# sekulas/vRod

Measured on AMD Instinct MI355X. Metric: queries/sec + recall@10 vs CPU ref, 10M×768 cosine, batch=1024, 1/2/4/8 GPU, higher is better.
Workload: dtype bf16

## Files before the change

### vrod_amd/csrc/kernels_select.hip

```cpp
#include "vrod_common.h"
#include "vrod_kernels.h"

namespace vrod {

constexpr int kSortThreads = 1024;

template <uint32_t NT = kSortThreads>
__device__ __forceinline__ void bitonic_sort_desc(uint64_t* __restrict__ a, uint32_t n) {
    const uint32_t tid = threadIdx.x, lane = tid & 63, wave = tid >> 6;
    constexpr uint32_t kWaves = NT / 64;
    const uint32_t W = n / 128 < kWaves ? (n / 128 ? n / 128 : 1) : kWaves;
    const uint32_t S = n / W;
    const bool active = wave < W;
    bool dirty_local = false;
    for (uint32_t k = 2; k <= n; k <<= 1) {
        for (uint32_t j = k >> 1; j > 0; j >>= 1) {
            if (j >= S) {
                if (dirty_local) { __syncthreads(); dirty_local = false; }
                for (uint32_t t = tid; t < (n >> 1); t += NT) {
                    const uint32_t i = 2 * t - (t & (j - 1));
                    const uint32_t l = i + j;
                    const bool up = (i & k) == 0;
                    const uint64_t x = a[i], y = a[l];
                    if ((x < y) == up) { a[i] = y; a[l] = x; }
                }
                __syncthreads();
            } else {
                if (active) {
                    const uint32_t base = wave * S;
                    for (uint32_t t = lane; t < (S >> 1); t += 64) {
                        const uint32_t i = base + 2 * t - (t & (j - 1));
                        const uint32_t l = i + j;
                        const bool up = (i & k) == 0;
                        const uint64_t x = a[i], y = a[l];
// ... 150 lines not shown
    const int lane = threadIdx.x & 63;
    for (uint32_t off = threadIdx.x; off < kCompactSlice; off += 256) {
        const uint64_t i = i0 + off;
        uint32_t skey = 0;
        bool take = false;
        if (i < n && !(row_mask && ((row_mask[i >> 5] >> (i & 31u)) & 1u))) {
            skey = score_key<METRIC>(sc[i]);
            take = skey >= thr_key;
        }
        const unsigned long long m = __ballot(take);
        if (m) {
            uint32_t base = 0;
            if (lane == 0) base = atomicAdd(&cnt[q], (uint32_t)__popcll(m));
            base = __shfl(base, 0);
            if (take) {
                const uint32_t pos = base + (uint32_t)__popcll(m & ((1ull << lane) - 1ull));
                if (pos < cap) keys[(uint64_t)q * cap + pos] = make_key(skey, (uint32_t)i);
            }
        }
    }
}

void launch_hist_compact(const float* d_scores, uint64_t score_ld, uint64_t n, int nq, int metric,
                         const uint32_t* d_hist, int hist_bits, uint32_t kp, uint64_t* d_keys,
                         uint32_t cap, uint32_t* d_cnt, uint32_t* d_status, const uint32_t* d_row_mask, hipStream_t s) {
    dim3 grid((unsigned)((n + kCompactSlice - 1) / kCompactSlice), nq);
    if (metric == M_COSINE)
        hist_compact_kernel<M_COSINE><<<grid, 256, 0, s>>>(d_scores, score_ld, n, d_hist, hist_bits, kp, d_keys, cap, d_cnt, d_status, d_row_mask);
    else
        hist_compact_kernel<M_L2><<<grid, 256, 0, s>>>(d_scores, score_ld, n, d_hist, hist_bits, kp, d_keys, cap, d_cnt, d_status, d_row_mask);
}

constexpr uint32_t kCompactThreads = 256;
__global__ __launch_bounds__(kCompactThreads) void list_compact_kernel(
    uint2* __restrict__ lists, uint32_t* __restrict__ counts, uint32_t cap, int metric,
    uint32_t keep, uint32_t wsize, float* __restrict__ thr, uint32_t* __restrict__ status,
    uint32_t* __restrict__ cand_rows, float* __restrict__ cand_fast, float* __restrict__ T) {
    extern __shared__ __attribute__((aligned(16))) uint64_t win[];
    const uint32_t q = blockIdx.x, tid = threadIdx.x;
    const uint32_t c = counts[q];
    const uint32_t n = c < cap ? c : cap;
    uint2* l = lists + (uint64_t)q * cap;
    const uint32_t kk = keep;
    uint32_t have = 0;
    uint32_t done = 0;
    while (done < n) {
        const uint32_t room = wsize - have;
        const uint32_t take = n - done < room ? n - done : room;
        for (uint32_t i = tid; i < take; i += kCompactThreads) {
            const uint2 e = l[done + i];
            win[have + i] = make_key(score_key_rt(__uint_as_float(e.x), metric), e.y);
        }
        const uint32_t m = have + take;
        const uint32_t np2 = pow2_ceil(m < 2 ? 2 : m);
        for (uint32_t i = m + tid; i < np2; i += kCompactThreads) win[i] = 0ull;
        __syncthreads();
        bitonic_sort_desc<kCompactThreads>(win, np2);
        have = m < kk ? m : kk;
        done += take;
        __syncthreads();
    }
    for (uint32_t i = tid; i < have; i += kCompactThreads) {
        const uint64_t key = win[i];
        l[i] = make_uint2(__float_as_uint(key_to_score_rt(key_skey(key), metric)), key_row(key));
    }
    if (cand_rows) {
        for (uint32_t i = tid; i < keep; i += kCompactThreads) {
            const uint64_t key = i < have ? win[i] : 0ull;
            cand_rows[(uint64_t)q * keep + i] = i < have ? key_row(key) : 0xFFFFFFFFu;
            cand_fast[(uint64_t)q * keep + i] = i < have ? key_to_score_rt(key_skey(key), metric) : __uint_as_float(kScoreNoneBits);
        }
    }
    if (tid == 0) {
        counts[q] = have;
        float t = thr[q];
        if (n >= keep && have >= keep) { t = key_to_score_rt(key_skey(win[keep - 1]), metric); thr[q] = t; }
        if (T) T[q] = t;
        if (c > cap) atomicOr(&status[q], 2u);
    }
}

void launch_list_compact(uint2* d_lists, uint32_t* d_counts, uint32_t cap, int nq, int metric,
                         uint32_t keep, float* d_thr, uint32_t* d_status, uint32_t* d_cand_rows,
                         float* d_cand_fast, float* d_T, hipStream_t s) {
    const uint32_t wsize = keep <= 1024 ? 2048u : kSelectChunk;
    list_compact_kernel<<<nq, kCompactThreads, (size_t)wsize * 8, s>>>(d_lists, d_counts, cap, metric, keep, wsize, d_thr, d_status,
                                                                     d_cand_rows, d_cand_fast, d_T);
}

constexpr uint32_t kSampleListCap = 2048;
template <int METRIC>
__global__ __launch_bounds__(256) void sample_select_kernel(const float* __restrict__ scores, uint64_t score_ld,
                                                            uint32_t n, uint32_t j, float* __restrict__ thr) {
    __shared__ __attribute__((aligned(16))) uint32_t hist[4096];
    __shared__ uint32_t ctl[8];
    const float* sc = scores + (uint64_t)blockIdx.x * score_ld;
    const uint32_t tid = threadIdx.x;
    if (j <= 256) {
        typedef float f4 __attribute__((ext_vector_type(4)));
        const f4 none4 = {__uint_as_float(kScoreNoneBits), __uint_as_float(kScoreNoneBits), __uint_as_float(kScoreNoneBits), __uint_as_float(kScoreNoneBits)};
        const uint32_t n4 = (n + 3) / 4;
        auto load4 = [&](uint32_t i4) -> f4 {
            if (i4 >= n4) return none4;
            f4 v = *reinterpret_cast<const f4*>(sc + (uint64_t)i4 * 4);
            if (i4 * 4 + 3 >= n) {
#pragma unroll
                for (int e = 0; e < 4; ++e) if (i4 * 4 + e >= n) v[e] = __uint_as_float(kScoreNoneBits);
            }
            return v;
        };
        uint32_t best = 0;
        for (uint32_t i0 = 0; i0 < n4; i0 += 256 * 8) {
// ... 89 lines not shown
    }
    if (lane == 0) thr[q] = key_to_score_rt(prefix, METRIC);
}

void launch_sample_select(const float* d_scores, uint64_t score_ld, uint32_t n_sample, int nq,
                          int metric, uint32_t j, float* d_thr, hipStream_t s) {
    if (!nq) return;
    if (n_sample <= kSampleWaveMax && j >= 1) {
        const int grid = (nq + 3) / 4;
        if (metric == M_COSINE) sample_select_wave_kernel<M_COSINE><<<grid, 256, 0, s>>>(d_scores, score_ld, n_sample, j, (uint32_t)nq, d_thr);
        else sample_select_wave_kernel<M_L2><<<grid, 256, 0, s>>>(d_scores, score_ld, n_sample, j, (uint32_t)nq, d_thr);
        return;
    }
    if (metric == M_COSINE) sample_select_kernel<M_COSINE><<<nq, 256, 0, s>>>(d_scores, score_ld, n_sample, j, d_thr);
    else sample_select_kernel<M_L2><<<nq, 256, 0, s>>>(d_scores, score_ld, n_sample, j, d_thr);
}

__global__ __launch_bounds__(256) void mask_sample_kernel(float* __restrict__ scores, uint64_t score_ld, uint32_t n, uint32_t nq,
                                                          uint64_t row0, const uint32_t* __restrict__ row_mask, float worst) {
    const uint32_t c = blockIdx.x * 256 + threadIdx.x;
    if (c >= n) return;
    const uint64_t r = row0 + c;
    if (!((row_mask[r >> 5] >> (r & 31u)) & 1u)) return;
    for (uint32_t q = blockIdx.y; q < nq; q += gridDim.y) scores[(uint64_t)q * score_ld + c] = worst;
}

void launch_mask_sample(float* d_scores, uint64_t score_ld, uint32_t n_sample, int nq, uint64_t row0,
                        const uint32_t* d_row_mask, int metric, hipStream_t s) {
    if (!nq || !n_sample || !d_row_mask) return;
    const dim3 grid((n_sample + 255) / 256, (unsigned)std::min(nq, 64));
    mask_sample_kernel<<<grid, 256, 0, s>>>(d_scores, score_ld, n_sample, (uint32_t)nq, row0, d_row_mask, worst_score(metric));
}

__global__ __launch_bounds__(kSortThreads) void final_topk_kernel(
    const uint32_t* __restrict__ cand_rows, const float* __restrict__ cand_fast,
    const float* __restrict__ cand_canon, const float* __restrict__ T, uint32_t kp, uint32_t k,
    int metric, IdMap idmap, int eps_mode, float eps_c, const uint32_t* __restrict__ max_qn2_bits,
    const uint32_t* __restrict__ max_xn2_bits, uint64_t* __restrict__ out_ids,
    float* __restrict__ out_scores, uint32_t* __restrict__ status, float* __restrict__ max_err) {
    extern __shared__ __attribute__((aligned(16))) uint64_t skeys[];
    const uint32_t q = blockIdx.x;
    const bool small = kp <= kRankSortMax;
    const uint32_t np2 = small ? kp : pow2_ceil(kp);
    float err = 0.0f;
    for (uint32_t i = threadIdx.x; i < np2; i += kSortThreads) {
        uint64_t key = 0;
        if (i < kp) {
            const uint32_t row = cand_rows[(uint64_t)q * kp + i];
            if (row != 0xFFFFFFFFu) {
                const float c = cand_canon[(uint64_t)q * kp + i];
                key = make_key(score_key_rt(c, metric), row);
                float e = __builtin_fabsf(cand_fast[(uint64_t)q * kp + i] - c);
                if (eps_mode == 1) e = e / __builtin_fmaxf(__builtin_fabsf(c), 1e-30f);
                if (e == e) err = __builtin_fmaxf(err, e);
            }
        }
        skeys[i] = key;
    }
    for (int o = 32; o > 0; o >>= 1) err = __builtin_fmaxf(err, __shfl_xor(err, o));
    if ((threadIdx.x & 63) == 0 && err > 0.0f) atomicMax((uint32_t*)max_err, __float_as_uint(err));
    __syncthreads();
    const uint64_t* sorted;
    if (small) {
        rank_sort_desc(skeys, skeys + kRankSortMax, np2);
        sorted = skeys + kRankSortMax;
    } else {
        bitonic_sort_desc(skeys, np2);
        sorted = skeys;
    }
    for (uint32_t i = threadIdx.x; i < k; i += kSortThreads) {
        const uint64_t key = i < np2 ? sorted[i] : 0ull;
        out_ids[(uint64_t)q * k + i] = key ? idmap(key_row(key)) : UINT64_MAX;
        out_scores[(uint64_t)q * k + i] = key ? key_to_score_rt(key_skey(key), metric) : __uint_as_float(kScoreNoneBits);
    }
    if (threadIdx.x == 0) {
        const float t = T[q];
        bool ok;
        const float qn_ = __builtin_sqrtf(__uint_as_float(*max_qn2_bits)), xn_ = __builtin_sqrtf(__uint_as_float(*max_xn2_bits));
        const float span = metric == M_COSINE ? qn_ * xn_ : (qn_ + xn_) * (qn_ + xn_);
        const float span_eps = eps_mode == 1 ? 0.0f : eps_c * span + eps_c * 2.3509887e-38f;
        if (!(span < 3.0e38f) || !(span + span_eps <= 3.4028234663852886e38f)) {
            ok = false;
        } else if (t == worst_score(metric)) {
            ok = true;
        } else {
            const uint64_t kk = (k >= 1 && k <= np2) ? sorted[k - 1] : 0ull;
            if (!kk) {
                ok = false;
            } else {
                const float sk = key_to_score_rt(key_skey(kk), metric);
                const float qn = __builtin_sqrtf(__uint_as_float(*max_qn2_bits));
                const float xn = __builtin_sqrtf(__uint_as_float(*max_xn2_bits));
                const float eps = (eps_mode == 0 ? eps_c * qn * xn
                                 : eps_mode == 1 ? eps_c * __builtin_fabsf(t) + 1e-30f
                                                 : eps_c * (qn + xn) * (qn + xn)) + eps_c * 2.3509887e-38f;
                ok = metric == M_COSINE ? (sk > t + eps) : (sk < t - eps);
            }
        }
        if (!ok) atomicOr(&status[q], 1u);
    }
}

void launch_final_topk(const uint32_t* d_cand_rows, const float* d_cand_fast,
                       const float* d_cand_canon, const float* d_T, int nq, uint32_t kp, uint32_t k,
                       int metric, const IdMap& idmap, int eps_mode, float eps_c,
                       const uint32_t* d_max_qn2_bits, const uint32_t* d_max_xn2_bits,
                       uint64_t* d_out_ids, float* d_out_scores, uint32_t* d_status,
                       float* d_max_err, hipStream_t s) {
    if (!nq) return;
    size_t lds = sort_lds_bytes(kp);
    if (lds < 2 * kRankSortMax * sizeof(uint64_t)) lds = 2 * kRankSortMax * sizeof(uint64_t);
    final_topk_kernel<<<nq, kSortThreads, lds, s>>>(d_cand_rows, d_cand_fast, d_cand_canon, d_T, kp, k, metric, idmap, eps_mode, eps_c, d_max_qn2_bits, d_max_xn2_bits, d_out_ids, d_out_scores, d_status, d_max_err);
}

__global__ __launch_bounds__(256) void gather_readback_kernel(const uint32_t* __restrict__ status, uint32_t nq,
                                                              uint32_t* __restrict__ flags3,
                                                              const uint32_t* __restrict__ max_xn2,
                                                              uint32_t* __restrict__ out) {
    for (uint32_t i = blockIdx.x * 256 + threadIdx.x; i < nq; i += gridDim.x * 256) out[i] = status[i];
    if (blockIdx.x == 0 && threadIdx.x < 4) {
        out[nq + threadIdx.x] = threadIdx.x < 3 ? flags3[threadIdx.x] : *max_xn2;
        if (threadIdx.x < 3) flags3[threadIdx.x] = 0;
    }
}

void launch_gather_readback(const uint32_t* d_status, uint32_t nq, uint32_t* d_flags3, const uint32_t* d_max_xn2,
                            uint32_t* d_out, hipStream_t s) {
    gather_readback_kernel<<<(nq + 255) / 256 > 0 ? (nq + 255) / 256 : 1, 256, 0, s>>>(d_status, nq, d_flags3, d_max_xn2, d_out);
}

__global__ __launch_bounds__(256) void band_prepare_kernel(const uint32_t* __restrict__ qidx, uint32_t nf, uint32_t nf_pad,
                                                           const float* __restrict__ out_scores, uint32_t k, int metric,
                                                           int eps_mode, float eps_c, const uint32_t* __restrict__ max_qn2_bits,
                                                           const uint32_t* __restrict__ max_xn2_bits, const float* __restrict__ qn2_all,
                                                           float* __restrict__ thr, float* __restrict__ qn2, uint32_t* __restrict__ counts,
                                                           uint32_t* __restrict__ ok) {
    const uint32_t f = blockIdx.x * 256 + threadIdx.x;
    if (f >= nf_pad) return;
    const float never = metric == M_COSINE ? __builtin_huge_valf() : -__builtin_huge_valf();
    counts[f] = 0u;
    if (f >= nf) { thr[f] = never; qn2[f] = 0.0f; ok[f] = 0u; return; }
    const uint32_t q = qidx[f];
    qn2[f] = qn2_all[q];
    const float ck = out_scores[(uint64_t)q * k + (k - 1)];
    const float qn = __builtin_sqrtf(__uint_as_float(*max_qn2_bits)), xn = __builtin_sqrtf(__uint_as_float(*max_xn2_bits));
    const float span = metric == M_COSINE ? qn * xn : (qn + xn) * (qn + xn);
    if (!(ck == ck) || !(span < 3.0e38f) || eps_mode == 1) { thr[f] = never; ok[f] = 0u; return; }
    const float eps = (eps_mode == 0 ? eps_c * qn * xn : eps_c * (qn + xn) * (qn + xn)) + eps_c * 2.3509887e-38f;
    const float slack = 1.01f * eps + 1e-37f;
    const float t = metric == M_COSINE ? ck - slack : ck + slack;
    if (!(span + eps <= 3.4028234663852886e38f) || !(__builtin_fabsf(t) <= 3.4028234663852886e38f)) { thr[f] = never; ok[f] = 0u; return; }
    thr[f] = t;
    ok[f] = 1u;
}

void launch_band_prepare(const uint32_t* d_qidx, uint32_t nf, uint32_t nf_pad, const float* d_out_scores, uint32_t k, int metric,
                         int eps_mode, float eps_c, const uint32_t* d_max_qn2_bits, const uint32_t* d_max_xn2_bits,
                         const float* d_qn2_all, float* d_thr, float* d_qn2, uint32_t* d_counts, uint32_t* d_ok, hipStream_t s) {
    if (!nf_pad) return;
    band_prepare_kernel<<<(nf_pad + 255) / 256, 256, 0, s>>>(d_qidx, nf, nf_pad, d_out_scores, k, metric, eps_mode, eps_c, d_max_qn2_bits,
                                                            d_max_xn2_bits, d_qn2_all, d_thr, d_qn2, d_counts, d_ok);
// ... 178 lines not shown
```

### vrod_amd/csrc/search_plan.h

```cpp
#pragma once
#include <stdint.h>

#include <algorithm>
#include <cmath>
#include <vector>

#include "../../include/vrod.h"

namespace vrod {

constexpr uint32_t kRowTile = 256;
constexpr uint32_t kSelectChunk = 8192;
enum : int { M_COSINE = 0, M_L2 = 1 };

inline uint64_t round_up(uint64_t x, uint64_t m) { return (x + m - 1) / m * m; }

inline int score_form(int metric) { return metric == VROD_METRIC_L2 ? M_L2 : M_COSINE; }
inline int prep_form(int metric) { return metric == VROD_METRIC_COSINE ? M_COSINE : M_L2; }

struct Route {
    int path;
    bool split;
};
inline bool can_split(bool split_enabled, int dtype, uint64_t N, uint32_t k) {
// ... 60 lines not shown
        }
    }
    return b;
}
inline float eps_bound(int eps_mode, float eps_c, float qn2, float xn2) {
    const float qn = std::sqrt(qn2), xn = std::sqrt(xn2);
    return (eps_mode == 0 ? eps_c * qn * xn : eps_mode == 1 ? eps_c  : eps_c * (qn + xn) * (qn + xn)) +
           (eps_mode == 1 ? 0.f : eps_c * 2.3509887e-38f);
}

struct SearchPlan {
    int path = 0;
    bool split = false;
    uint32_t kp = 0;
    int eps_mode = 0;
    float eps_c = 0.f;
    uint32_t nq_pad = 0;
    uint64_t N = 0;
};
inline SearchPlan make_plan(int path, bool split, int form, uint32_t dim, uint64_t N, uint32_t nq, uint32_t k, uint32_t kp_boost,
                            uint32_t kp_margin) {
    SearchPlan p;
    p.path = path;
    p.split = split;
    p.kp = choose_kp(path, split, form, N, k, kp_boost, kp_margin);
    const FastBound b = fast_bound(path, split, form, dim);
    p.eps_mode = b.mode;
    p.eps_c = b.c;
    p.nq_pad = (uint32_t)round_up(nq, path == VROD_PATH_MFMA ? 256 : 8);
    p.N = N;
    return p;
}

struct StagePlan { uint32_t S, j; std::vector<uint64_t> bounds; };
inline StagePlan plan_stages(uint64_t N, uint32_t kp, uint32_t cap, uint32_t max_sample_rows, uint64_t stage_growth,
                             uint64_t sample_rows) {
    StagePlan p;
    const uint64_t g_auto = 5;
    const uint64_t g = std::max<uint64_t>(2, std::min<uint64_t>(stage_growth ? stage_growth : g_auto, cap / (3ull * kp)));
    if (sample_rows) max_sample_rows = (uint32_t)std::min<uint64_t>(sample_rows, max_sample_rows);
    uint64_t S = std::min<uint64_t>(N / (g * g), max_sample_rows);
    S = std::max<uint64_t>(S, std::min<uint64_t>(N, std::max<uint64_t>(4ull * kp, kRowTile)));
    S = std::min<uint64_t>(round_up(S, kRowTile), N);
    p.S = (uint32_t)S;
    p.j = (uint32_t)std::min<uint64_t>(kp, S);
    for (uint64_t b = S * g; b < N; b *= g) {
        if (N - b < b / 2) break;
        p.bounds.push_back(b / kRowTile * kRowTile);
    }
    p.bounds.push_back(N);
    return p;
}

struct KpBoost {
    static constexpr uint32_t kMax = 8;
    uint32_t boost = 1, clean = 0, hold = 0;
};
inline void kp_boost_step(KpBoost& s, uint32_t used, bool failures) {
    if (s.hold) --s.hold;
    if (failures) {
        s.clean = 0;
        if (used >= KpBoost::kMax) { s.boost = 1; s.hold = 256; }
        else if (!s.hold && used == s.boost) s.boost *= 2;
    } else if (used == s.boost && ++s.clean >= 64 && s.boost > 1) {
        s.boost /= 2;
        s.clean = 0;
// ... 65 lines not shown
```

### vrod_amd/csrc/vrod_index.hip

```cpp
#include <hip/hip_runtime.h>
#include <dlfcn.h>
#include <fcntl.h>
#include <unistd.h>
#include <rccl/rccl.h>

#include <algorithm>
#include <cmath>
#include <cstdarg>
#include <cstdio>
#include <cstdlib>
#include <cstring>
#include <string>
#include <vector>

#include "../../include/vrod.h"
#include "vrod_common.h"
#include "vrod_kernels.h"
#include "kernels_range.h"
#include "search_plan.h"
#include "compact_plan.h"
#include "label_plan.h"
#include "group_plan.h"
#include "byid_plan.h"

// ... 49 lines not shown
};

constexpr uint32_t kPaceRegions = 8, kPaceWords = 192, kClaimWords = (uint32_t)kMfmaClaimWords;
constexpr size_t kSlotFlagBytes = (64 + kPaceRegions * (kPaceWords + kClaimWords)) * 4;

struct Pending {
    bool active = false;
    bool trivial = false;
    uint32_t nq = 0, k = 0;
    SearchPlan plan{};
    uint64_t* out_ids = nullptr;
    float* out_scores = nullptr;
    hipStream_t stream = nullptr;
    uint32_t* flags = nullptr;
    DevBuf q_raw, q_lp, scores, keys_a, keys_b, lists, small, hist, cand_rows, cand_fast, cand_canon;
    DevBuf q_f32;
    DevBuf dump;
    DevBuf q_planes;
    DevBuf band_idx, band_q, band_q_lp, band_planes, band_small, band_ids, band_scores;
    uint32_t pace_launches = 0;
    uint32_t* h_readback = nullptr;
    size_t h_readback_words = 0;
    hipEvent_t done = nullptr;
    hipEvent_t scans_done = nullptr;
    hipEvent_t mid_done = nullptr;
    bool mid_recorded = false;
    std::vector<hipEvent_t> ev;
    size_t ev_used = 0, t0 = 0, t1 = 0;
    std::vector<std::pair<size_t, size_t>> scan_pairs;
    int sample_pair = -1;
    int tail_pair = -1;
    uint32_t seq = 0;
    bool early_sample = false;
    uint32_t kp_boost_used = 1;
    vrod_search_stats st{};

    struct GraphKey {
        const void *q = nullptr, *oi = nullptr, *os = nullptr, *corpus = nullptr, *xn = nullptr, *mask = nullptr;
        const void* bufs[12] = {};
        uint64_t N = 0, id_offset = 0;
        uint32_t nq = 0, k = 0;
        int path = 0;
        bool operator==(const GraphKey& o) const { return memcmp(this, &o, sizeof *this) == 0; }
    };
    GraphKey gkey{};
    bool gkey_valid = false;
    hipGraphExec_t gexec = nullptr;
    GraphKey gkey_graph{};
    bool graph_off = false;
    SearchPlan g_plan{};
    vrod_search_stats g_st{};
};

struct vrod_index {
    int device = 0;
    int num_cus = 256;
    uint32_t dim = 0, ld = 0;
    int dtype = VROD_DTYPE_F32, metric = VROD_METRIC_COSINE;
    size_t esize = 4;
    uint64_t count = 0, capacity = 0, id_offset = 0;
    void* corpus = nullptr;
    float* xnorm2 = nullptr;
    uint32_t* max_xn2_bits = nullptr;
    hipStream_t stream = nullptr;
    int path = VROD_PATH_AUTO;
    int profiling = 0;
// ... 332 lines not shown
    if (e == hipSuccess) { launch_xn2_max(idx->xnorm2, plan.live, idx->max_xn2_bits, s); e = hipGetLastError(); }
    if (e == hipSuccess) e = hipMemsetAsync(idx->del_dev, 0, cap_words * 4, s);
    if (e == hipSuccess && idx->filter_on) e = hipMemcpyAsync(idx->eff_dev, new_eff.data(), cap_words * 4, hipMemcpyHostToDevice, s);
    if (e == hipSuccess && idx->lab_dev) e = hipMemcpyAsync(idx->lab_dev, new_lab.data(), count * 4, hipMemcpyHostToDevice, s);
    if (e == hipSuccess) e = hipStreamSynchronize(s);
    if (e != hipSuccess)
        return fail(VROD_ERR_HIP, "vrod_index_compact: %s while rows were moving: the handle is unusable, destroy it", hipGetErrorString(e));

    if (out_new_ids) compact_new_ids(del, count, idx->id_offset, out_new_ids);
    std::fill(idx->del_bits.begin(), idx->del_bits.end(), 0u);
    idx->n_deleted = 0;
    idx->count = plan.live;
    if (idx->filter_on) { idx->allow_bits.swap(new_allow); idx->eff_bits.swap(new_eff); }
    if (idx->lab_dev) std::copy(new_lab.begin(), new_lab.end(), idx->lab_bits.begin());
    idx->planes_rows = 0;
    mask_changed(idx);
    return VROD_OK;
}

namespace vrod {
const DebugEnv& debug_env() {
    static const DebugEnv env = [] {
        DebugEnv d;
        auto num = [](const char* name, long long dflt) { const char* e = getenv(name); return e && *e ? atoll(e) : dflt; };
        auto on = [](const char* name) { const char* e = getenv(name); return !e || e[0] != '0'; };
        d.pace_kt = (int)num("VROD_DEBUG_PACE_KT", d.pace_kt);
        d.pace_tiles = (int)num("VROD_DEBUG_PACE", d.pace_tiles);
        d.w4_steal = on("VROD_DEBUG_W4_STEAL");
        d.skinny = on("VROD_DEBUG_SKINNY");
        d.stage_growth = (uint64_t)num("VROD_DEBUG_STAGE_GROWTH", 0);
        d.sample_rows = (uint64_t)num("VROD_DEBUG_SAMPLE_ROWS", 0);
        d.kp_margin = (uint32_t)num("VROD_DEBUG_KP_MARGIN", 0);
        if (const char* e = getenv("VROD_DEBUG_EARLY_SAMPLE")) d.early_sample = e[0] != '0' ? 1 : 0;
        d.sample_grouped = on("VROD_DEBUG_SAMPLE_GROUPED");
        d.graph = on("VROD_DEBUG_GRAPH");
        d.band = on("VROD_DEBUG_BAND");
        return d;
    }();
    return env;
}
}

struct Timer {
    vrod_index* idx;
    Pending& P;
    Timer(vrod_index* i, Pending& p) : idx(i), P(p) {}
    size_t mark() {
        if (idx->profiling < 2) return 0;
        if (P.ev_used == P.ev.size()) {
            hipEvent_t e;
            if (hipEventCreate(&e) != hipSuccess) return 0;
            P.ev.push_back(e);
        }
        (void)hipEventRecord(P.ev[P.ev_used], P.stream);
        return P.ev_used++;
    }
    void arm(size_t& a, size_t& b) {
        a = b = 0;
        if (!idx->profiling) return;
        while (P.ev.size() < P.ev_used + 2) {
            hipEvent_t e;
            if (hipEventCreate(&e) != hipSuccess) return;
            P.ev.push_back(e);
        }
        a = P.ev_used++;
        b = P.ev_used++;
// ... 266 lines not shown
            tm.arm(a, b);
            g_launch_events = LaunchEvents{};
            if (b) HIP_TRY(hipEventRecord(P.ev[a], s));
        }
        launch_rescore_list(idx->corpus, idx->dtype, form, idx->dim, idx->ld, P.q_f32.as<float>() + (size_t)q0 * idx->ld, gc, list, m,
                            P.scores.as<float>(), score_ld, s);
        if (idx->profiling && b) {
            HIP_TRY(hipEventRecord(P.ev[b], s));
            P.scan_pairs.push_back({a, b});
        }
        st.scan_launches++;
        const uint64_t* keys; uint64_t kld, kn;
        VROD_TRY(select_chain(idx, P, P.scores.as<float>(), score_ld, m, (int)gc, kx, nullptr, &keys, &kld, &kn));
        launch_list_keys_to_output(keys, kld, kn, (int)gc, form, k, list, idmap_of(idx), P.out_ids + (size_t)q0 * k,
                                   P.out_scores + (size_t)q0 * k, s);
    }
    VROD_TRY(record_scans_done(P, s));
    st.scan_bytes = (double)m * idx->ld * idx->esize;
    st.scan_flops = 2.0 * nq * (double)m * idx->dim;
    HIP_TRY(hipGetLastError());
    return VROD_OK;
}

static int mfma_pass(vrod_index* idx, Pending& P, Timer& tm, const void* q_lp) {
    const SearchPlan& plan = P.plan;
    const uint64_t N = plan.N;
    const uint32_t nq = P.nq, kp = plan.kp, cap = kSelectChunk;
    const int form = score_form(idx->metric);
    const SmallBlock B = small_block(P);
    const ListBlock L = list_block(P);
    vrod_search_stats& st = P.st;
    hipStream_t s = P.stream;
    const int early_env = debug_env().early_sample;
    const bool early = early_env >= 0 ? early_env == 1 : N <= 6000000ull;
    Pending& O = other_slot(idx, P);
    HIP_TRY(hipStreamWaitEvent(s, early ? O.mid_done : O.scans_done, 0));
    MfmaScanArgs a;
    VROD_TRY(mfma_args(idx, P, a, idx->dtype == VROD_DTYPE_BF16 ? q_lp : P.q_f32.p, B.qn2, B.thr, nq, plan.nq_pad));
    if (plan.split) {
        if (idx->planes_rows < N) {
            launch_split_rows((const float*)idx->corpus + idx->planes_rows * idx->ld, N - idx->planes_rows, idx->ld, idx->ldp,
                              (char*)idx->planes + idx->planes_rows * 2ull * idx->ldp * 2ull, false, s);
            if (round_up(N, kRowTile) > N)
                HIP_TRY(hipMemsetAsync((char*)idx->planes + N * 2ull * idx->ldp * 2ull, 0, (round_up(N, kRowTile) - N) * 2ull * idx->ldp * 2ull, s));
            idx->planes_rows = N;
        }
        VROD_TRY(use_split_planes(idx, a, P.q_f32.as<float>(), plan.nq_pad, P.q_planes, s));
    }
    const int scan_dtype = plan.split ? VROD_DTYPE_BF16 : idx->dtype;
    P.pace_launches = 0;
    std::vector<uint64_t> bounds{N};
    if (N > cap) {
        const uint32_t nqb = plan.nq_pad / 256;
        const StagePlan sp = plan_stages(N, kp, cap, std::max<uint32_t>(1, (uint32_t)idx->num_cus / nqb) * kRowTile,
                                         debug_env().stage_growth, debug_env().sample_rows);
        bounds = sp.bounds;
        MfmaScanArgs d = a;
        const uint64_t w0 = sample_window(idx, sp.S, N);
        d.row_begin = (uint32_t)w0; d.row_end = (uint32_t)(w0 + sp.S);
        const bool group_env = debug_env().sample_grouped && !idx->row_mask();
        const uint32_t grows = group_env ? mfma_dense_group_rows(d, scan_dtype) : 0u;
        const uint32_t n_groups = grows ? (uint32_t)(round_up(sp.S, kRowTile) / grows) : 0u;
        const bool grouped = grows && (uint64_t)sp.j * 8 <= n_groups && sp.S % kRowTile == 0;
        const uint32_t dense_ld = grouped ? (uint32_t)round_up(n_groups, 64) : (uint32_t)round_up(sp.S, kRowTile);
        const uint32_t n_sel = grouped ? n_groups : sp.S;
        VROD_TRY(P.scores.ensure((size_t)plan.nq_pad * dense_ld * 4));
        d.dense_out = P.scores.as<float>(); d.dense_ld = dense_ld; d.dense_grouped = grouped;
        d.pace = pace_region(P, P.pace_launches++); d.pace_is_zero = true;
        size_t e0, e1;
        tm.arm(e0, e1);
        launch_scan_mfma(d, scan_dtype, idx->num_cus, s);
        P.sample_pair = (int)P.scan_pairs.size();
        P.early_sample = early;
        P.scan_pairs.push_back({e0, e1});
        st.scan_launches++;
        launch_mask_sample(P.scores.as<float>(), dense_ld, n_sel, (int)nq, w0, idx->row_mask(), form, s);
        launch_sample_select(P.scores.as<float>(), dense_ld, n_sel, (int)nq, form, sp.j, B.thr, s);
    }
    HIP_TRY(hipStreamWaitEvent(s, early ? O.scans_done : O.done, 0));
    uint64_t lo = 0;
    for (size_t li = 0; li < bounds.size(); ++li) {
        const bool last = li + 1 == bounds.size();
        launch_filtered(idx, P, tm, a, scan_dtype, lo, bounds[li], true, last);
        lo = std::max(lo, bounds[li]);
        if (li + 2 == bounds.size()) { HIP_TRY(hipEventRecord(P.mid_done, s)); P.mid_recorded = true; }
        if (last) VROD_TRY(record_scans_done(P, s));
        launch_list_compact(L.lists, L.counts, cap, (int)nq, form, kp, B.thr, B.status, last ? P.cand_rows.as<uint32_t>() : nullptr,
                            last ? P.cand_fast.as<float>() : nullptr, last ? B.T : nullptr, s);
    }
    HIP_TRY(hipGetLastError());
    return VROD_OK;
}

static int search_enqueue_body(vrod_index* idx, Pending& P, const float* d_queries_raw, uint32_t nq, uint32_t k,
                               uint64_t* d_out_ids, float* d_out_scores, bool in_graph) {
    vrod_search_stats& st = P.st;
    st = vrod_search_stats{};
    st.nq = nq;
    st.k = k;
    P.nq = nq; P.k = k; P.out_ids = d_out_ids; P.out_scores = d_out_scores;
    P.trivial = true;
    P.mid_recorded = false;
    P.ev_used = 0; P.t0 = P.t1 = 0; P.scan_pairs.clear(); P.sample_pair = -1;
    P.tail_pair = -1; P.early_sample = false; P.seq = idx->n_begun;
    idx->tail_ev[P.seq & 3].armed = false;
    if (!nq) return VROD_OK;
    hipStream_t s = P.stream;
    Timer tm(idx, P);
    P.t0 = tm.mark();

    const uint64_t N = idx->count;
    const int form = score_form(idx->metric);
    const bool gather = !idx->mask_ovr && (idx->path == VROD_PATH_GATHER || (idx->filter_on && filter_route(idx->path, idx->dtype, N, idx->eligible(), nq, idx->dim)));
    Route r = gather ? Route{VROD_PATH_GATHER, false}
                     : route(idx->path, idx->dtype, idx->split_enabled, mfma_skinny_max_queries(true, 2u * idx->ldp * 2u), N, nq, k);
    if (r.split && !planes_ready(idx)) r.split = false;
    P.plan = make_plan(r.path, r.split, form, idx->dim, N, nq, k, idx->kp_boost.boost, debug_env().kp_margin);
    const SearchPlan& plan = P.plan;
    P.kp_boost_used = idx->kp_boost.boost;
    st.kprime = gather ? 0u : plan.kp;
    st.path = plan.path;
    st.split_pass = plan.split ? 1u : 0u;

    if (N == 0 || idx->eligible() == 0) {
        std::vector<uint64_t> hi((size_t)nq * k, UINT64_MAX);
        std::vector<uint32_t> hs((size_t)nq * k, kScoreNoneBits);
        HIP_TRY(hipMemcpyAsync(d_out_ids, hi.data(), hi.size() * 8, hipMemcpyHostToDevice, s));
        HIP_TRY(hipMemcpyAsync(d_out_scores, hs.data(), hs.size() * 4, hipMemcpyHostToDevice, s));
        HIP_TRY(hipStreamSynchronize(s));
        return VROD_OK;
    }

    const uint32_t nq_pad = plan.nq_pad;
    const bool mfma = plan.path == VROD_PATH_MFMA;
    P.trivial = false;
    if (!P.done) HIP_TRY(hipEventCreateWithFlags(&P.done, hipEventDisableTiming));
    VROD_TRY(P.q_f32.ensure((size_t)nq_pad * idx->ld * 4));
    void* q_lp = nullptr;
    if (idx->dtype == VROD_DTYPE_BF16) {
        VROD_TRY(P.q_lp.ensure((size_t)nq_pad * idx->ld * 2));
        q_lp = P.q_lp.p;
    }
    VROD_TRY(P.small.ensure(small_bytes(nq_pad)));
    if (P.h_readback_words < (size_t)nq + 4) {
        if (P.h_readback) (void)hipHostFree(P.h_readback);
        P.h_readback = nullptr;
        P.h_readback_words = 0;
        HIP_TRY(hipHostMalloc((void**)&P.h_readback, ((size_t)nq + 4 + 1024) * 4, hipHostMallocDefault));
        P.h_readback_words = (size_t)nq + 4 + 1024;
    }
    if (mfma) VROD_TRY(P.lists.ensure(list_bytes(nq_pad)));
    const SmallBlock B = small_block(P);
    const uint32_t worst_bits = form == M_COSINE ? 0xFF800000u : 0x7F800000u;
    QueryInit qi{};
    qi.status = B.status;
    qi.counts = mfma ? list_block(P).counts : nullptr;
    qi.thr = mfma ? B.thr : nullptr;
    qi.thr_live_bits = worst_bits;
    qi.thr_pad_bits = worst_bits ^ 0x80000000u;
    qi.zero_words = nullptr;
    qi.n_zero_words = 0;
    qi.zero_words2 = mfma ? pace_region(P, 0) : nullptr;
    qi.n_zero_words2 = kPaceRegions * (kPaceWords + kClaimWords);
    if (plan.path == VROD_PATH_STREAM) {
        VROD_TRY(P.hist.ensure(kHistWords * 4));
        qi.zero_words2 = P.hist.as<uint32_t>();
        qi.n_zero_words2 = (uint32_t)kHistWords;
    }
    launch_prep_queries(d_queries_raw, nq, nq_pad, idx->dim, idx->ld, idx->prep_ovr >= 0 ? idx->prep_ovr : prep_form(idx->metric), idx->dtype,
                        P.q_f32.as<float>(), q_lp, B.qn2, &P.flags[0], &P.flags[1], qi, s);
    HIP_TRY(hipGetLastError());

    VROD_TRY(P.cand_rows.ensure((size_t)nq * plan.kp * 4));
    VROD_TRY(P.cand_fast.ensure((size_t)nq * plan.kp * 4));
    VROD_TRY(P.cand_canon.ensure((size_t)nq * plan.kp * 4));
    if (plan.path == VROD_PATH_STREAM) VROD_TRY(stream_pass(idx, P, tm, in_graph));
    else if (mfma) VROD_TRY(mfma_pass(idx, P, tm, q_lp));
    else if (gather) VROD_TRY(gather_pass(idx, P, tm));

    if (plan.path != VROD_PATH_EXACT && !gather) {
        launch_rescore_candidates(idx->corpus, idx->dtype, form, idx->dim, idx->ld, P.q_f32.as<float>(), (int)nq,
                                  P.cand_rows.as<uint32_t>(), plan.kp, P.cand_canon.as<float>(), s);
        launch_final_topk(P.cand_rows.as<uint32_t>(), P.cand_fast.as<float>(), P.cand_canon.as<float>(), B.T, (int)nq, plan.kp, k,
                          form, idmap_of(idx), plan.eps_mode, plan.eps_c, &P.flags[1], idx->max_xn2_bits, d_out_ids, d_out_scores,
                          B.status, (float*)&P.flags[2], s);
    }
    launch_gather_readback(B.status, nq, P.flags, idx->max_xn2_bits, B.readback, s);
    HIP_TRY(hipGetLastError());
    HIP_TRY(hipMemcpyAsync(P.h_readback, B.readback, ((size_t)nq + 4) * 4, hipMemcpyDeviceToHost, s));
    P.t1 = tm.mark();
    if (!in_graph) HIP_TRY(hipEventRecord(P.done, s));
    return VROD_OK;
}

static int search_enqueue(vrod_index* idx, Pending& P, const float* d_queries_raw, uint32_t nq, uint32_t k,
                          uint64_t* d_out_ids, float* d_out_scores) {
    const bool graphs_on = debug_env().graph;
    const uint64_t N = idx->count;
    const bool gather = !idx->mask_ovr && (idx->path == VROD_PATH_GATHER || (idx->filter_on && filter_route(idx->path, idx->dtype, N, idx->eligible(), nq, idx->dim)));
    const bool graphable = graphs_on && idx->prep_ovr < 0 && !P.graph_off && idx->profiling == 0 && nq >= 1 && nq <= 8 && idx->eligible() > 0 && idx->n_pending() >= 1 &&
                           !gather && graph_route(idx->path, nq) && (double)N * idx->ld * idx->esize <= 64.0 * 1048576.0;
    Pending::GraphKey key{};
    if (graphable) {
        key.q = d_queries_raw; key.oi = d_out_ids; key.os = d_out_scores; key.corpus = idx->corpus; key.xn = idx->xnorm2;
        key.mask = idx->row_mask();
        const void* bufs[12] = {P.q_f32.p, P.q_lp.p, P.small.p, P.hist.p, P.scores.p, P.keys_a.p, P.cand_rows.p, P.cand_fast.p,
                                P.cand_canon.p, P.h_readback, P.flags, idx->max_xn2_bits};
        memcpy(key.bufs, bufs, sizeof bufs);
        key.N = N; key.id_offset = idmap_of(idx).offset; key.nq = nq; key.k = k; key.path = idx->path;
    }
    Pending& O = other_slot(idx, P);
    hipStream_t s = P.stream;
    if (graphable && P.gexec && P.gkey_graph == key) {
        P.st = P.g_st;
        P.nq = nq; P.k = k; P.out_ids = d_out_ids; P.out_scores = d_out_scores;
        P.trivial = false; P.ev_used = 0; P.t0 = P.t1 = 0; P.scan_pairs.clear();
        P.plan = P.g_plan;
        HIP_TRY(hipStreamWaitEvent(s, O.scans_done, 0));
        HIP_TRY(hipGraphLaunch(P.gexec, s));
        P.mid_recorded = false;
// ... 2098 lines not shown
```

### vrod_amd/csrc/vrod_kernels.h

```cpp
#pragma once
#include <hip/hip_runtime.h>
#include <hip/hip_ext.h>
#include <stdint.h>

#include "search_plan.h"
#include "label_plan.h"

namespace vrod {

struct IdMap {
    uint64_t offset = 0;
    uint32_t block_rows = 0;
    uint32_t shard = 0, n_shards = 1;
    __host__ __device__ inline uint64_t operator()(uint32_t row) const {
        if (block_rows == 0) return (uint64_t)row + offset;
        const uint64_t b = row / block_rows, r = row % block_rows;
        return (b * n_shards + shard) * block_rows + r + offset;
    }
};

void launch_synth_rows(uint64_t seed, uint64_t first_row, uint64_t n, uint32_t dim, float* d_out,
                       hipStream_t s);
void launch_prepare_rows(const float* d_in, uint64_t n, uint32_t dim, uint32_t ld, int metric,
                         int dtype, double* d_nrm_ws, uint32_t* d_bad_flag, float* d_out_f32,
// ... 28 lines not shown

void launch_scan_stream(const void* d_corpus, int dtype, int metric, uint32_t ld, uint64_t nrows,
                        const float* d_q, int nq_pad, float* d_scores, uint64_t score_ld,
                        uint32_t* d_hist, uint32_t kp, const uint32_t* d_row_mask, hipStream_t s);
int stream_hist_bits(int nq_pad);
int stream_max_queries_per_pass(uint32_t ld);
void launch_hist_compact(const float* d_scores, uint64_t score_ld, uint64_t n, int nq, int metric,
                         const uint32_t* d_hist, int hist_bits, uint32_t kp, uint64_t* d_keys,
                         uint32_t cap, uint32_t* d_cnt, uint32_t* d_status, const uint32_t* d_row_mask,
                         hipStream_t s);

uint64_t launch_select_from_scores(const float* d_scores, uint64_t score_ld, uint64_t n, int nq,
                                   int metric, uint32_t kp, uint64_t* d_out, uint64_t out_ld,
                                   const uint32_t* d_row_mask, hipStream_t s, const uint32_t* d_len = nullptr);
uint64_t launch_select_from_keys(const uint64_t* d_in, uint64_t in_ld, uint64_t n, int nq,
                                 uint32_t kp, uint64_t* d_out, uint64_t out_ld, hipStream_t s);
void launch_keys_to_candidates(const uint64_t* d_keys, uint64_t key_ld, uint64_t n, int nq,
                               int metric, uint32_t kp, uint32_t* d_cand_rows, float* d_cand_fast,
                               float* d_T, const uint32_t* d_cnt, hipStream_t s);

void launch_list_compact(uint2* d_lists, uint32_t* d_counts, uint32_t cap, int nq, int metric,
                         uint32_t keep, float* d_thr, uint32_t* d_status, uint32_t* d_cand_rows,
                         float* d_cand_fast, float* d_T, hipStream_t s);
void launch_sample_select(const float* d_scores, uint64_t score_ld, uint32_t n_sample, int nq,
                          int metric, uint32_t j, float* d_thr, hipStream_t s);
void launch_mask_sample(float* d_scores, uint64_t score_ld, uint32_t n_sample, int nq, uint64_t row0,
                        const uint32_t* d_row_mask, int metric, hipStream_t s);
void launch_final_topk(const uint32_t* d_cand_rows, const float* d_cand_fast,
                       const float* d_cand_canon, const float* d_T, int nq, uint32_t kp, uint32_t k,
                       int metric, const IdMap& idmap, int eps_mode, float eps_c,
                       const uint32_t* d_max_qn2_bits, const uint32_t* d_max_xn2_bits,
                       uint64_t* d_out_ids, float* d_out_scores, uint32_t* d_status,
                       float* d_max_err, hipStream_t s);

void launch_band_prepare(const uint32_t* d_qidx, uint32_t nf, uint32_t nf_pad, const float* d_out_scores, uint32_t k, int metric,
                         int eps_mode, float eps_c, const uint32_t* d_max_qn2_bits, const uint32_t* d_max_xn2_bits,
                         const float* d_qn2_all, float* d_thr, float* d_qn2, uint32_t* d_counts, uint32_t* d_ok, hipStream_t s);
void launch_gather_query_rows(const float* d_src, const uint32_t* d_qidx, uint32_t nf, uint32_t nf_pad, uint32_t ld, float* d_dst_f32,
                              void* d_dst_bf16, hipStream_t s);
void launch_scatter_results(const uint64_t* d_ids, const float* d_scores, const uint32_t* d_qidx, const uint32_t* d_resolved, uint32_t nf,
                            uint32_t k, uint64_t* d_out_ids, float* d_out_scores, hipStream_t s);

void launch_keys_to_output(const uint64_t* d_keys, uint64_t n, int metric, uint32_t k,
                           const IdMap& idmap, uint64_t* d_out_ids, float* d_out_scores,
                           hipStream_t s);
void launch_list_keys_to_output(const uint64_t* d_keys, uint64_t key_ld, uint64_t n, int nq, int metric, uint32_t k,
                                const uint32_t* d_list, const IdMap& idmap, uint64_t* d_out_ids, float* d_out_scores,
                                hipStream_t s);

void launch_seg_keys_to_output(const uint64_t* d_keys, uint64_t key_ld, uint64_t n, int ns, int metric, uint32_t k,
                               const uint32_t* d_lists, const uint32_t* d_seg_base, const uint32_t* d_slot_q, const IdMap& idmap,
                               uint64_t* d_out_ids, float* d_out_scores, hipStream_t s);

void launch_fill_none(uint64_t* d_ids, float* d_scores, uint64_t n, hipStream_t s);
void launch_merge_topk(int metric, const uint64_t* d_ids, const float* d_scores, uint64_t list_stride_ids,
                       uint64_t list_stride_scores, uint32_t n_lists, uint32_t nq, uint32_t k,
                       uint64_t* d_out_ids, float* d_out_scores, hipStream_t s);

void launch_rescore_candidates(const void* d_corpus, int dtype, int metric, uint32_t dim,
                               uint32_t ld, const float* d_q, int nq, const uint32_t* d_cand_rows,
                               uint32_t kp, float* d_out, hipStream_t s);
int rescore_all_max_queries(uint32_t ld);
void launch_rescore_all(const void* d_corpus, int dtype, int metric, uint32_t dim, uint32_t ld,
                        const float* d_q, const uint32_t* query_index, int nq, uint64_t nrows,
                        float* d_out, uint64_t out_ld, hipStream_t s);
void launch_rescore_list(const void* d_corpus, int dtype, int metric, uint32_t dim, uint32_t ld, const float* d_q, uint32_t nq,
// ... 36 lines not shown
    const float* thr;
    uint2* lists;
    uint32_t* counts;
    uint32_t cap;
    uint32_t ld;
    uint32_t lda_bytes;
    uint32_t a_wrap;
    uint32_t nq_pad;
    uint32_t nq;
    uint32_t row_begin;
    uint32_t row_end;
    int metric;
    uint32_t* pace;
    bool pace_is_zero;
    float* dense_out;
    uint32_t dense_ld;
    bool dense_grouped;
    void* dump;
    uint32_t* claims;
    bool claims_is_zero;
    const uint32_t* row_mask;
};
void launch_scan_mfma(const MfmaScanArgs& a, int dtype, int num_cus, hipStream_t s);

struct DebugEnv {
    int pace_kt = 192;
    int pace_tiles = 16;
    bool w4_steal = true;
    bool skinny = true;
    uint64_t stage_growth = 0;
    uint64_t sample_rows = 0;
    uint32_t kp_margin = 0;
    int early_sample = -1;
    bool sample_grouped = true;
    bool graph = true;
    bool band = true;
};
const DebugEnv& debug_env();
size_t mfma_dump_bytes(int num_cus);
constexpr size_t kMfmaClaimWords = 256;
uint32_t mfma_dense_group_rows(const MfmaScanArgs& a, int dtype);
uint32_t mfma_skinny_max_queries(bool split, uint32_t row_bytes);

}
```

Measured before the change: 89160.

## Fuse list compaction, rescoring, final top-k and readback into one tail kernel

Adds an optional tail kernel that runs the final list compaction, the canonical rescoring of candidates, the rank sort and the certificate check per query in one work-group. A ticket counter lets the last group write the readback flags, replacing several separate launches. It is gated by a debug env flag that defaults to off. Separately, the early-sample overlap now defaults on for all corpus sizes instead of only small ones, which changes which event the next batch's scan waits on.

```diff
diff --git a/vrod_amd/csrc/kernels_select.hip b/vrod_amd/csrc/kernels_select.hip
--- a/vrod_amd/csrc/kernels_select.hip
+++ b/vrod_amd/csrc/kernels_select.hip
@@ -1,5 +1,6 @@
 #include "vrod_common.h"
 #include "vrod_kernels.h"
+#include "rescore_chain.h"
 
 namespace vrod {
 
@@ -216,12 +217,11 @@
 }
 
 constexpr uint32_t kCompactThreads = 256;
-__global__ __launch_bounds__(kCompactThreads) void list_compact_kernel(
-    uint2* __restrict__ lists, uint32_t* __restrict__ counts, uint32_t cap, int metric,
+__device__ __forceinline__ uint32_t list_compact_body(
+    uint64_t* win, uint32_t q, uint2* __restrict__ lists, uint32_t* __restrict__ counts, uint32_t cap, int metric,
     uint32_t keep, uint32_t wsize, float* __restrict__ thr, uint32_t* __restrict__ status,
-    uint32_t* __restrict__ cand_rows, float* __restrict__ cand_fast, float* __restrict__ T) {
-    extern __shared__ __attribute__((aligned(16))) uint64_t win[];
-    const uint32_t q = blockIdx.x, tid = threadIdx.x;
+    uint32_t* __restrict__ cand_rows, float* __restrict__ cand_fast, float* __restrict__ T, float* t_out) {
+    const uint32_t tid = threadIdx.x;
     const uint32_t c = counts[q];
     const uint32_t n = c < cap ? c : cap;
     uint2* l = lists + (uint64_t)q * cap;
@@ -261,7 +261,18 @@
         if (n >= keep && have >= keep) { t = key_to_score_rt(key_skey(win[keep - 1]), metric); thr[q] = t; }
         if (T) T[q] = t;
         if (c > cap) atomicOr(&status[q], 2u);
-    }
+        *t_out = t;
+    }
+    return have;
+}
+
+__global__ __launch_bounds__(kCompactThreads) void list_compact_kernel(
+    uint2* __restrict__ lists, uint32_t* __restrict__ counts, uint32_t cap, int metric,
+    uint32_t keep, uint32_t wsize, float* __restrict__ thr, uint32_t* __restrict__ status,
+    uint32_t* __restrict__ cand_rows, float* __restrict__ cand_fast, float* __restrict__ T) {
+    extern __shared__ __attribute__((aligned(16))) uint64_t win[];
+    float t;
+    (void)list_compact_body(win, blockIdx.x, lists, counts, cap, metric, keep, wsize, thr, status, cand_rows, cand_fast, T, &t);
 }
 
 void launch_list_compact(uint2* d_lists, uint32_t* d_counts, uint32_t cap, int nq, int metric,
@@ -417,6 +428,40 @@
     mask_sample_kernel<<<grid, 256, 0, s>>>(d_scores, score_ld, n_sample, (uint32_t)nq, row0, d_row_mask, worst_score(metric));
 }
 
+__device__ __forceinline__ uint64_t cand_key(uint32_t row, float c, float fast, int metric, int eps_mode, float& err) {
+    float e = __builtin_fabsf(fast - c);
+    if (eps_mode == 1) e = e / __builtin_fmaxf(__builtin_fabsf(c), 1e-30f);
+    if (e == e) err = __builtin_fmaxf(err, e);
+    return make_key(score_key_rt(c, metric), row);
+}
+__device__ __forceinline__ bool certificate_ok(float t, const uint64_t* sorted, uint32_t np2, uint32_t k, int metric, int eps_mode,
+                                               float eps_c, const uint32_t* __restrict__ max_qn2_bits,
+                                               const uint32_t* __restrict__ max_xn2_bits) {
+    bool ok;
+    const float qn_ = __builtin_sqrtf(__uint_as_float(*max_qn2_bits)), xn_ = __builtin_sqrtf(__uint_as_float(*max_xn2_bits));
+    const float span = metric == M_COSINE ? qn_ * xn_ : (qn_ + xn_) * (qn_ + xn_);
+    const float span_eps = eps_mode == 1 ? 0.0f : eps_c * span + eps_c * 2.3509887e-38f;
+    if (!(span < 3.0e38f) || !(span + span_eps <= 3.4028234663852886e38f)) {
+        ok = false;
+    } else if (t == worst_score(metric)) {
+        ok = true;
+    } else {
+        const uint64_t kk = (k >= 1 && k <= np2) ? sorted[k - 1] : 0ull;
+        if (!kk) {
+            ok = false;
+        } else {
+            const float sk = key_to_score_rt(key_skey(kk), metric);
+            const float qn = __builtin_sqrtf(__uint_as_float(*max_qn2_bits));
+            const float xn = __builtin_sqrtf(__uint_as_float(*max_xn2_bits));
+            const float eps = (eps_mode == 0 ? eps_c * qn * xn
+                             : eps_mode == 1 ? eps_c * __builtin_fabsf(t) + 1e-30f
+                                             : eps_c * (qn + xn) * (qn + xn)) + eps_c * 2.3509887e-38f;
+            ok = metric == M_COSINE ? (sk > t + eps) : (sk < t - eps);
+        }
+    }
+    return ok;
+}
+
 __global__ __launch_bounds__(kSortThreads) void final_topk_kernel(
     const uint32_t* __restrict__ cand_rows, const float* __restrict__ cand_fast,
     const float* __restrict__ cand_canon, const float* __restrict__ T, uint32_t kp, uint32_t k,
@@ -433,11 +478,7 @@
         if (i < kp) {
             const uint32_t row = cand_rows[(uint64_t)q * kp + i];
             if (row != 0xFFFFFFFFu) {
-                const float c = cand_canon[(uint64_t)q * kp + i];
-                key = make_key(score_key_rt(c, metric), row);
-                float e = __builtin_fabsf(cand_fast[(uint64_t)q * kp + i] - c);
-                if (eps_mode == 1) e = e / __builtin_fmaxf(__builtin_fabsf(c), 1e-30f);
-                if (e == e) err = __builtin_fmaxf(err, e);
+                key = cand_key(row, cand_canon[(uint64_t)q * kp + i], cand_fast[(uint64_t)q * kp + i], metric, eps_mode, err);
             }
         }
         skeys[i] = key;
@@ -459,29 +500,7 @@
         out_scores[(uint64_t)q * k + i] = key ? key_to_score_rt(key_skey(key), metric) : __uint_as_float(kScoreNoneBits);
     }
     if (threadIdx.x == 0) {
-        const float t = T[q];
-        bool ok;
-        const float qn_ = __builtin_sqrtf(__uint_as_float(*max_qn2_bits)), xn_ = __builtin_sqrtf(__uint_as_float(*max_xn2_bits));
-        const float span = metric == M_COSINE ? qn_ * xn_ : (qn_ + xn_) * (qn_ + xn_);
-        const float span_eps = eps_mode == 1 ? 0.0f : eps_c * span + eps_c * 2.3509887e-38f;
-        if (!(span < 3.0e38f) || !(span + span_eps <= 3.4028234663852886e38f)) {
-            ok = false;
-        } else if (t == worst_score(metric)) {
-            ok = true;
-        } else {
-            const uint64_t kk = (k >= 1 && k <= np2) ? sorted[k - 1] : 0ull;
-            if (!kk) {
-                ok = false;
-            } else {
-                const float sk = key_to_score_rt(key_skey(kk), metric);
-                const float qn = __builtin_sqrtf(__uint_as_float(*max_qn2_bits));
-                const float xn = __builtin_sqrtf(__uint_as_float(*max_xn2_bits));
-                const float eps = (eps_mode == 0 ? eps_c * qn * xn
-                                 : eps_mode == 1 ? eps_c * __builtin_fabsf(t) + 1e-30f
-                                                 : eps_c * (qn + xn) * (qn + xn)) + eps_c * 2.3509887e-38f;
-                ok = metric == M_COSINE ? (sk > t + eps) : (sk < t - eps);
-            }
-        }
+        const bool ok = certificate_ok(T[q], sorted, np2, k, metric, eps_mode, eps_c, max_qn2_bits, max_xn2_bits);
         if (!ok) atomicOr(&status[q], 1u);
     }
 }
@@ -512,6 +531,97 @@
 void launch_gather_readback(const uint32_t* d_status, uint32_t nq, uint32_t* d_flags3, const uint32_t* d_max_xn2,
                             uint32_t* d_out, hipStream_t s) {
     gather_readback_kernel<<<(nq + 255) / 256 > 0 ? (nq + 255) / 256 : 1, 256, 0, s>>>(d_status, nq, d_flags3, d_max_xn2, d_out);
+}
+
+constexpr uint32_t kTailThreads = kCompactThreads;
+constexpr uint32_t kTailWindow = 2048;
+static_assert(kTailFusedMaxKp <= 64 && kTailFusedMaxKp <= kRankSortMax && 2 * kTailFusedMaxKp <= kTailWindow, "one lane per candidate");
+constexpr size_t kTailWorkBytes = (size_t)64 * kTileStride * 4 + 2 * kRankSortMax * 8;
+static_assert((size_t)kTailWindow * 8 <= kTailWorkBytes && kTailFusedMaxDim * 4 + kTailWorkBytes <= 65536, "LDS of one work-group");
+template <typename T, int METRIC, bool COMPACT>
+__global__ __launch_bounds__(kTailThreads) void tail_fused_kernel(const TailArgs a) {
+    extern __shared__ __attribute__((aligned(16))) float tail_lds[];
+    __shared__ float t_lds;
+    float* q_lds = tail_lds;
+    uint64_t* win = reinterpret_cast<uint64_t*>(tail_lds + a.ld);
+    float* tile = tail_lds + a.ld;
+    uint64_t* skeys = reinterpret_cast<uint64_t*>(tile + 64 * kTileStride);
+    const uint32_t q = blockIdx.x, tid = threadIdx.x, kp = a.kp, k = a.k;
+    const float* qrow = a.q + (uint64_t)q * a.ld;
+    for (uint32_t i = tid; i < a.ld; i += kTailThreads) q_lds[i] = qrow[i];
+
+    uint32_t row = 0xFFFFFFFFu;
+    float fast = __uint_as_float(kScoreNoneBits);
+    if constexpr (COMPACT) {
+        float t = 0.0f;
+        const uint32_t have = list_compact_body(win, q, a.lists, a.counts, a.cap, METRIC, kp, kTailWindow, a.thr, a.status, a.cand_rows,
+                                                a.cand_fast, a.T, &t);
+        if (tid < kp && tid < have) {
+            const uint64_t key = win[tid];
+            row = key_row(key);
+            fast = key_to_score_rt(key_skey(key), METRIC);
+        }
+        if (tid == 0) t_lds = t;
+    } else {
+        if (tid < kp) {
+            row = a.cand_rows[(uint64_t)q * kp + tid];
+            fast = a.cand_fast[(uint64_t)q * kp + tid];
+        }
+        if (tid == 0) t_lds = a.T[q];
+    }
+    __syncthreads();
+
+    if (tid < 64) {
+        const bool valid = row != 0xFFFFFFFFu;
+        const unsigned long long vmask = __ballot(valid);
+        float canon = __uint_as_float(kScoreNoneBits);
+        if (vmask != 0ull) {
+            const float acc = canonical_chain_wave<T, METRIC>((const T*)a.corpus, a.dim, a.ld, q_lds, tile, valid ? row : 0u,
+                                                              64 - __builtin_clzll(vmask));
+            if (valid) canon = acc;
+        }
+        float err = 0.0f;
+        uint64_t key = 0ull;
+        if (valid) key = cand_key(row, canon, fast, METRIC, a.eps_mode, err);
+        for (int o = 32; o > 0; o >>= 1) err = __builtin_fmaxf(err, __shfl_xor(err, o));
+        if (tid == 0 && err > 0.0f) atomicMax(&a.flags[2], __float_as_uint(err));
+        if (tid < kp) {
+            a.cand_canon[(uint64_t)q * kp + tid] = canon;
+            skeys[tid] = key;
+        }
+    }
+    __syncthreads();
+    rank_sort_desc(skeys, skeys + kRankSortMax, kp);
+    const uint64_t* sorted = skeys + kRankSortMax;
+    for (uint32_t i = tid; i < k; i += kTailThreads) {
+        const uint64_t key = i < kp ? sorted[i] : 0ull;
+        a.out_ids[(uint64_t)q * k + i] = key ? a.idmap(key_row(key)) : UINT64_MAX;
+        a.out_scores[(uint64_t)q * k + i] = key ? key_to_score_rt(key_skey(key), METRIC) : __uint_as_float(kScoreNoneBits);
+    }
+    if (tid == 0) {
+        const bool ok = certificate_ok(t_lds, sorted, kp, k, METRIC, a.eps_mode, a.eps_c, &a.flags[1], a.max_xn2_bits);
+        const uint32_t bit = ok ? 0u : 1u;
+        a.readback[q] = atomicOr(&a.status[q], bit) | bit;
+        __threadfence();
+        if (atomicAdd(&a.flags[kTailTicketWord], 1u) == a.nq - 1u) {
+            __threadfence();
+            for (uint32_t i = 0; i < 3; ++i) a.readback[a.nq + i] = atomicExch(&a.flags[i], 0u);
+            a.readback[a.nq + 3] = *a.max_xn2_bits;
+            atomicExch(&a.flags[kTailTicketWord], 0u);
+        }
+    }
+}
+
+void launch_tail_fused(const TailArgs& a, int dtype, int metric, hipStream_t s) {
+    if (!a.nq) return;
+    const bool compact = a.lists != nullptr;
+    const size_t lds = (size_t)a.ld * 4 + kTailWorkBytes;
+#define VROD_TF(TT, MM, CC) tail_fused_kernel<TT, MM, CC><<<a.nq, kTailThreads, lds, s>>>(a)
+#define VROD_TF_C(TT, MM) do { if (compact) VROD_TF(TT, MM, true); else VROD_TF(TT, MM, false); } while (0)
+    if (dtype == DT_BF16) { if (metric == M_COSINE) VROD_TF_C(bf16_t, M_COSINE); else VROD_TF_C(bf16_t, M_L2); }
+    else { if (metric == M_COSINE) VROD_TF_C(float, M_COSINE); else VROD_TF_C(float, M_L2); }
+#undef VROD_TF_C
+#undef VROD_TF
 }
 
 __global__ __launch_bounds__(256) void band_prepare_kernel(const uint32_t* __restrict__ qidx, uint32_t nf, uint32_t nf_pad,
diff --git a/vrod_amd/csrc/search_plan.h b/vrod_amd/csrc/search_plan.h
--- a/vrod_amd/csrc/search_plan.h
+++ b/vrod_amd/csrc/search_plan.h
@@ -116,6 +116,12 @@
     return p;
 }
 
+constexpr uint32_t kTailFusedMaxKp = 64, kTailFusedMaxDim = 8192;
+inline bool tail_fused(const SearchPlan& p, uint32_t nq, uint32_t dim, bool enabled) {
+    return enabled && nq > 0 && p.kp >= 1 && p.kp <= kTailFusedMaxKp && dim <= kTailFusedMaxDim &&
+           (p.path == VROD_PATH_STREAM || p.path == VROD_PATH_MFMA);
+}
+
 struct StagePlan { uint32_t S, j; std::vector<uint64_t> bounds; };
 inline StagePlan plan_stages(uint64_t N, uint32_t kp, uint32_t cap, uint32_t max_sample_rows, uint64_t stage_growth,
                              uint64_t sample_rows) {
diff --git a/vrod_amd/csrc/vrod_index.hip b/vrod_amd/csrc/vrod_index.hip
--- a/vrod_amd/csrc/vrod_index.hip
+++ b/vrod_amd/csrc/vrod_index.hip
@@ -105,6 +105,7 @@
     int tail_pair = -1;
     uint32_t seq = 0;
     bool early_sample = false;
+    bool tail_fused = false;
     uint32_t kp_boost_used = 1;
     vrod_search_stats st{};
 
@@ -503,6 +504,7 @@
         d.sample_rows = (uint64_t)num("VROD_DEBUG_SAMPLE_ROWS", 0);
         d.kp_margin = (uint32_t)num("VROD_DEBUG_KP_MARGIN", 0);
         if (const char* e = getenv("VROD_DEBUG_EARLY_SAMPLE")) d.early_sample = e[0] != '0' ? 1 : 0;
+        d.tail_fused = num("VROD_DEBUG_TAIL_FUSED", 0) != 0;
         d.sample_grouped = on("VROD_DEBUG_SAMPLE_GROUPED");
         d.graph = on("VROD_DEBUG_GRAPH");
         d.band = on("VROD_DEBUG_BAND");
@@ -835,7 +837,7 @@
     vrod_search_stats& st = P.st;
     hipStream_t s = P.stream;
     const int early_env = debug_env().early_sample;
-    const bool early = early_env >= 0 ? early_env == 1 : N <= 6000000ull;
+    const bool early = early_env != 0;
     Pending& O = other_slot(idx, P);
     HIP_TRY(hipStreamWaitEvent(s, early ? O.mid_done : O.scans_done, 0));
     MfmaScanArgs a;
@@ -888,6 +890,7 @@
         lo = std::max(lo, bounds[li]);
         if (li + 2 == bounds.size()) { HIP_TRY(hipEventRecord(P.mid_done, s)); P.mid_recorded = true; }
         if (last) VROD_TRY(record_scans_done(P, s));
+        if (last && P.tail_fused) break;
         launch_list_compact(L.lists, L.counts, cap, (int)nq, form, kp, B.thr, B.status, last ? P.cand_rows.as<uint32_t>() : nullptr,
                             last ? P.cand_fast.as<float>() : nullptr, last ? B.T : nullptr, s);
     }
@@ -924,6 +927,7 @@
     st.kprime = gather ? 0u : plan.kp;
     st.path = plan.path;
     st.split_pass = plan.split ? 1u : 0u;
+    P.tail_fused = tail_fused(plan, nq, idx->dim, debug_env().tail_fused && !gather && !idx->mask_ovr && idx->prep_ovr < 0);
 
     if (N == 0 || idx->eligible() == 0) {
         std::vector<uint64_t> hi((size_t)nq * k, UINT64_MAX);
@@ -981,14 +985,25 @@
     else if (mfma) VROD_TRY(mfma_pass(idx, P, tm, q_lp));
     else if (gather) VROD_TRY(gather_pass(idx, P, tm));
 
-    if (plan.path != VROD_PATH_EXACT && !gather) {
+    if (P.tail_fused) {
+        TailArgs t{};
+        if (mfma) { const ListBlock L = list_block(P); t.lists = L.lists; t.counts = L.counts; t.cap = kSelectChunk; t.thr = B.thr; }
+        t.corpus = idx->corpus; t.dim = idx->dim; t.ld = idx->ld; t.q = P.q_f32.as<float>();
+        t.cand_rows = P.cand_rows.as<uint32_t>(); t.cand_fast = P.cand_fast.as<float>(); t.cand_canon = P.cand_canon.as<float>(); t.T = B.T;
+        t.nq = nq; t.kp = plan.kp; t.k = k;
+        t.idmap = idmap_of(idx);
+        t.eps_mode = plan.eps_mode; t.eps_c = plan.eps_c;
+        t.flags = P.flags; t.max_xn2_bits = idx->max_xn2_bits;
+        t.out_ids = d_out_ids; t.out_scores = d_out_scores; t.status = B.status; t.readback = B.readback;
+        launch_tail_fused(t, idx->dtype, form, s);
+    } else if (plan.path != VROD_PATH_EXACT && !gather) {
         launch_rescore_candidates(idx->corpus, idx->dtype, form, idx->dim, idx->ld, P.q_f32.as<float>(), (int)nq,
                                   P.cand_rows.as<uint32_t>(), plan.kp, P.cand_canon.as<float>(), s);
         launch_final_topk(P.cand_rows.as<uint32_t>(), P.cand_fast.as<float>(), P.cand_canon.as<float>(), B.T, (int)nq, plan.kp, k,
                           form, idmap_of(idx), plan.eps_mode, plan.eps_c, &P.flags[1], idx->max_xn2_bits, d_out_ids, d_out_scores,
                           B.status, (float*)&P.flags[2], s);
     }
-    launch_gather_readback(B.status, nq, P.flags, idx->max_xn2_bits, B.readback, s);
+    if (!P.tail_fused) launch_gather_readback(B.status, nq, P.flags, idx->max_xn2_bits, B.readback, s);
     HIP_TRY(hipGetLastError());
     HIP_TRY(hipMemcpyAsync(P.h_readback, B.readback, ((size_t)nq + 4) * 4, hipMemcpyDeviceToHost, s));
     P.t1 = tm.mark();
diff --git a/vrod_amd/csrc/vrod_kernels.h b/vrod_amd/csrc/vrod_kernels.h
--- a/vrod_amd/csrc/vrod_kernels.h
+++ b/vrod_amd/csrc/vrod_kernels.h
@@ -84,6 +84,19 @@
                        const uint32_t* d_max_qn2_bits, const uint32_t* d_max_xn2_bits,
                        uint64_t* d_out_ids, float* d_out_scores, uint32_t* d_status,
                        float* d_max_err, hipStream_t s);
+
+constexpr uint32_t kTailTicketWord = 5;
+struct TailArgs {
+    uint2* lists; uint32_t* counts; uint32_t cap; float* thr;
+    const void* corpus; uint32_t dim, ld; const float* q;
+    uint32_t* cand_rows; float* cand_fast; float* cand_canon; float* T;
+    uint32_t nq, kp, k;
+    IdMap idmap;
+    int eps_mode; float eps_c;
+    uint32_t* flags; const uint32_t* max_xn2_bits;
+    uint64_t* out_ids; float* out_scores; uint32_t* status; uint32_t* readback;
+};
+void launch_tail_fused(const TailArgs& a, int dtype, int metric, hipStream_t s);
 
 void launch_band_prepare(const uint32_t* d_qidx, uint32_t nf, uint32_t nf_pad, const float* d_out_scores, uint32_t k, int metric,
                          int eps_mode, float eps_c, const uint32_t* d_max_qn2_bits, const uint32_t* d_max_xn2_bits,
@@ -186,6 +199,7 @@
     uint64_t sample_rows = 0;
     uint32_t kp_margin = 0;
     int early_sample = -1;
+    bool tail_fused = false;
     bool sample_grouped = true;
     bool graph = true;
     bool band = true;
```

Result: no change. 89680 (median of 6 runs) (+0.6%).
